# harskish/ganspace

Hardware: NVIDIA H100
Metric: latent samples/sec into PCA (StyleGAN2-ffhq W, N=1e6) (higher is better)
Workload: dtype f32

## Files before the change

### ganspace_b200/_native.py

```python
from __future__ import annotations

import contextlib
import ctypes as C
import os
from pathlib import Path

import torch

_LIB_PATH = Path(__file__).resolve().parent / "libganspace_b200.so"
_lib = None

_P, _I, _L, _Z, _D, _F = C.c_void_p, C.c_int, C.c_int64, C.c_size_t, C.c_double, C.c_float
SIGNATURES = {
    "gsb_abi_version": (_I, []),
    "gsb_last_error": (C.c_char_p, []),
    "gsb_legacy_normal_f32": (_I, [_P, _I, _L, _P, _L, _P]),
    "gsb_legacy_truncnorm_f32": (_I, [_P, _I, _L, _D, _D, _F, _P, _L, _P]),
    "gsb_mt19937_raw_u32": (_I, [_P, _I, _L, _P, _L, _P]),
    "gsb_mt19937_jump_polys": (_I, [_L, _I, _P]),
    "gsb_mt19937_jump_state_host": (_I, [C.c_uint32, _P, _P]),
    "gsb_legacy_normal_split_step_words": (_L, [_L, _I]),
    "gsb_legacy_normal_split_workspace_bytes": (_Z, [_I, _L, _I]),
    "gsb_legacy_normal_f32_split": (_I, [_P, _I, _L, _P, _L, _I, _P, _P, _Z, _P]),
    "gsb_legacy_normal_split_status": (_I, [_P, _I, _L, _I, _P, _P]),
    "gsb_mapping_packed_bytes": (_Z, [_I, _I]),
    "gsb_mapping_pack": (_I, [_P, _P, _I, _I, _F, _P, _P]),
    "gsb_mapping_workspace_bytes": (_Z, [_L, _I]),
    "gsb_mapping_forward": (_I, [_P, _I, _I, _P, _P, _L, _I, _P, _Z, _P]),
    "gsb_mapping_status": (_I, [_P, _I, _I, _P]),
    "gsb_linear_forward": (_I, [_P, _P, _P, _P, _L, _I, _I, _I, _P, _Z, _P]),
    "gsb_linear_workspace_bytes": (_Z, [_L, _I, _I, _I]),
    "gsb_batch_stats_workspace_bytes": (_Z, [_L, _I]),
    "gsb_batch_stats": (_I, [_P, _L, _I, _L, _P, _P, _P, _Z, _P]),
    "gsb_batch_stats_multi_workspace_bytes": (_Z, [_I, _L, _I]),
    "gsb_batch_stats_multi": (_I, [_P, _I, _L, _I, _L, _P, _P, _P, _Z, _P]),
    "gsb_ipca_state_bytes": (_Z, [_I, _I]),
    "gsb_ipca_workspace_bytes": (_Z, [_I, _I]),
    "gsb_ipca_reset": (_I, [_P, _I, _I, _P]),
    "gsb_ipca_chain_step": (_I, [_P, _I, _I, _L, _L, _P, _P, _P, _Z, _P]),
    "gsb_ipca_export": (_I, [_P, _I, _I, _L, _P, _P, _P, _P, _P, _P, _P]),
    "gsb_sym_eig_top": (_I, [_P, _I, _I, _P, _P, _P, _Z, _P]),
    "gsb_eig_status": (_I, [_P, _P]),
    "gsb_project_std_workspace_bytes": (_Z, [_I]),
    "gsb_project_std": (_I, [_P, _L, _I, _L, _P, _I, _P, _P, _P, _Z, _P]),
    "gsb_linreg_state_bytes": (_Z, [_I, _I]),
    "gsb_linreg_reset": (_I, [_P, _I, _I, _P]),
    "gsb_linreg_workspace_bytes": (_Z, [_L, _I]),
    "gsb_linreg_accumulate": (_I, [_P, _I, _I, _P, _L, _I, _P, _P, _P, _P, _P, _Z, _P]),
    "gsb_linreg_solve": (_I, [_P, _I, _I, _L, _P, _P, _P]),
    "gsb_linreg_solve_status": (_I, [_P, _I, _I, _P, _P]),
    "gsb_linreg_normal_matrix": (_P, [_P, _I, _I]),
    "gsb_linreg_solve_pinv": (_I, [_P, _I, _I, _P, _P, _D, _P, _P]),
    "gsb_ipca_set_chain_mode": (_I, [_I]),
    "gsb_synthesis_packed_bytes": (_Z, [_P, _I, _I]),
    "gsb_synthesis_pack": (_I, [_P, _I, _I, _P, _P, _Z, _P]),
    "gsb_synthesis_workspace_bytes": (_Z, [_P, _I, _L]),
    "gsb_synthesis_forward": (_I, [_P, _P, _I, _I, _I, _P, _L, _P, _L, _P, _Z, _P]),
    "gsb_synthesis_status": (_I, [_P, _P, _I, _I, _P]),
    "gsb_synthesis_render_workspace_bytes": (_Z, [_P, _I, _L, _I]),
    "gsb_synthesis_render": (_I, [_P, _P, _I, _I, _I, _P, _I, _P, _I, _L, _P, _L, _P, _P, _Z, _P]),
    "gsb_bigd_rows": (_I, [_I, _I]),
    "gsb_bigd_state_bytes": (_Z, [_L, _I]),
# ... 359 lines not shown
    return mean_out, gram_out


def batch_stats_multi(x: torch.Tensor, n_groups: int, rows_per_group: int, mean_out: torch.Tensor = None,
                      gram_out: torch.Tensor = None):
    lib = load()
    assert x.is_cuda and x.dtype == torch.float32 and x.dim() == 2 and x.stride(1) == 1
    assert x.shape[0] >= n_groups * rows_per_group
    d, ld = x.shape[1], x.stride(0)
    mean = mean_out if mean_out is not None else torch.empty((n_groups, d), dtype=torch.float64, device=x.device)
    gram = gram_out if gram_out is not None else torch.empty((n_groups, d, d), dtype=torch.float64, device=x.device)
    assert mean.shape == (n_groups, d) and gram.shape == (n_groups, d, d) and mean.dtype == gram.dtype == torch.float64
    ws_bytes = lib.gsb_batch_stats_multi_workspace_bytes(n_groups, rows_per_group, d)
    ws = scratch.get("stats", ws_bytes, x.device)
    with torch.cuda.device(x.device), instrument.section("stats"):
        _check(lib.gsb_batch_stats_multi(C.c_void_p(x.data_ptr()), n_groups, rows_per_group, d, ld, _ptr(mean), _ptr(gram),
                                         _ptr(ws), ws.numel(), _stream()), "gsb_batch_stats_multi")
    instrument.count(4 if (d % 128 == 0 and d <= 1024) else 3 * n_groups)
    return mean, gram


class IPCAChain:

    def __init__(self, d: int, c: int, device, side_stream: bool = True):
        lib = load()
        self.dev = require_cuda(device)
        self.d, self.c = int(d), int(c)
        self.state = torch.empty(lib.gsb_ipca_state_bytes(self.d, self.c), dtype=torch.uint8, device=self.dev)
        self.ws = torch.empty(lib.gsb_ipca_workspace_bytes(self.d, self.c), dtype=torch.uint8, device=self.dev)
        self.n_seen = 0
        self.stream = None
        if side_stream and os.environ.get("GANSPACE_B200_CHAIN_STREAM", "1") != "0":
            with torch.cuda.device(self.dev):
                self.stream = torch.cuda.Stream(device=self.dev, priority=-1)
        with torch.cuda.device(self.dev):
            _check(lib.gsb_ipca_reset(_ptr(self.state), self.d, self.c, _stream()), "gsb_ipca_reset")
            if self.stream is not None:
                self.stream.wait_stream(torch.cuda.current_stream())

    def step(self, n_batch: int, mean_b: torch.Tensor, gram_b: torch.Tensor):
        lib = load()
        assert mean_b.dtype == torch.float64 and gram_b.dtype == torch.float64
        with torch.cuda.device(self.dev):
            if self.stream is not None:
                self.stream.wait_stream(torch.cuda.current_stream())
                mean_b.record_stream(self.stream)
                gram_b.record_stream(self.stream)
                ctx = torch.cuda.stream(self.stream)
            else:
                ctx = contextlib.nullcontext()
            with ctx, instrument.section("chain"):
                _check(lib.gsb_ipca_chain_step(_ptr(self.state), self.d, self.c, self.n_seen, int(n_batch),
                                               _ptr(mean_b), _ptr(gram_b), _ptr(self.ws), self.ws.numel(), _stream()),
                       "gsb_ipca_chain_step")
        subspace = (self.d % 128 == 0 and 128 <= self.d <= 512 and self.c % 8 == 0 and 8 <= self.c <= 128
                    and os.environ.get("GANSPACE_B200_CHAIN", "") != "direct" and not _chain_forced_direct)
        instrument.count((1 if self.n_seen > 0 else 9) if subspace else 8)
        self.n_seen += int(n_batch)

    def join(self):
        if self.stream is not None:
            with torch.cuda.device(self.dev):
                torch.cuda.current_stream().wait_stream(self.stream)

    def export(self):
        lib = load()
        self.join()
        f64 = dict(dtype=torch.float64, device=self.dev)
        out = {
            "components": torch.empty((self.c, self.d), **f64), "singular_values": torch.empty(self.c, **f64),
            "mean": torch.empty(self.d, **f64), "var": torch.empty(self.d, **f64),
            "explained_variance": torch.empty(self.c, **f64),
            "explained_variance_ratio": torch.empty(self.c, **f64),
        }
        with torch.cuda.device(self.dev):
            _check(lib.gsb_ipca_export(_ptr(self.state), self.d, self.c, self.n_seen, _ptr(out["components"]),
                                       _ptr(out["singular_values"]), _ptr(out["mean"]), _ptr(out["var"]),
                                       _ptr(out["explained_variance"]), _ptr(out["explained_variance_ratio"]),
                                       _stream()), "gsb_ipca_export")
            check_eig_status("IPCAChain.export")
        instrument.count(1)
# ... 395 lines not shown
```

### ganspace_b200/csrc/ipca.cu

```cuda
#include "ipca_internal.cuh"
#include <math.h>

namespace gsb {

constexpr int ST_HDR = 24;

struct StateView {
    double *hdr, *mean, *unnorm, *S, *V;
    double *H, *Qbuf;
    void *eig_ws;
    size_t bytes;
};
static inline size_t export_eig_n(int c) { return (size_t)(c + 31) / 32 * 32; }
inline StateView state_view(void *p, int d, int c) {
    StateView s;
    s.hdr = reinterpret_cast<double *>(p);
    s.mean = s.hdr + ST_HDR;
    s.unnorm = s.mean + d;
    s.S = s.unnorm + d;
    s.V = s.S + c;
    size_t off = align_up((size_t)(ST_HDR + 2 * (size_t)d + c + (size_t)c * d) * sizeof(double), 256);
    s.H = s.Qbuf = nullptr; s.eig_ws = nullptr;
    if (subspace_applicable(d, c)) {
        char *b = reinterpret_cast<char *>(p);
// ... 129 lines not shown
extern "C" int gsb_ipca_chain_step(void *d_state, int d, int c, int64_t n_seen, int64_t n_batch,
                                   const double *d_mean_b, const double *d_gram_b, void *d_workspace,
                                   size_t workspace_bytes, gsb_stream_t stream) {
    GSB_CHECK_ARG(d_state && d_mean_b && d_gram_b && d_workspace, "ipca_chain_step: null pointer");
    if (int r = gsb::check_dims(d, c)) return r;
    GSB_CHECK_ARG(n_seen >= 0 && n_batch > 0, "ipca_chain_step: bad counts");
    GSB_CHECK_ARG(n_seen > 0 || c <= n_batch, "ipca_chain_step: n_components=%d > first batch size %lld", c,
                  (long long)n_batch);
    gsb::Workspace w = gsb::carve(d_workspace, d, c);
    if (workspace_bytes < w.bytes) {
        gsb::set_error("ipca_chain_step: workspace too small (%zu < %zu)", workspace_bytes, w.bytes);
        return GSB_ERR_WORKSPACE;
    }
    cudaStream_t st = (cudaStream_t)stream;
    gsb::StateView s = gsb::state_view(d_state, d, c);
    const bool subspace = gsb::subspace_applicable(d, c);
    if (subspace && n_seen > 0) {
        const size_t off = w.bytes;
        gsb::SubspaceWs sw = gsb::carve_subspace(reinterpret_cast<char *>(d_workspace) + off, d, c);
        if (workspace_bytes < off + sw.bytes) {
            gsb::set_error("ipca_chain_step: workspace too small (%zu < %zu)", workspace_bytes, off + sw.bytes);
            return GSB_ERR_WORKSPACE;
        }
        return gsb::subspace_step(s.hdr, s.mean, s.unnorm, s.H, s.Qbuf, d_mean_b, d_gram_b, sw, d, c, (double)n_seen,
                                  (double)n_batch, st);
    }
    dim3 grid((d + 31) / 32, (d + 31) / 32), block(32, 8);
    gsb::build_g_kernel<<<grid, block, 0, st>>>(d_gram_b, d_mean_b, s.mean, s.S, s.V, d, c, (double)n_seen,
                                                (double)n_batch, w.A);
    GSB_CHECK_LAUNCH();
    if (int r = gsb::eig_top(w, d, c, w.lam, w.evecs, st)) return r;
    size_t tot = (size_t)c * d;
    gsb::finalize_kernel<<<(unsigned)((tot + 255) / 256), 256, 0, st>>>(
        s.hdr, s.mean, s.unnorm, s.S, s.V, d_mean_b, d_gram_b, w.lam, w.evecs, d, c, (double)n_seen,
        (double)n_batch);
    GSB_CHECK_LAUNCH();
    if (subspace) return gsb::to_subspace_form(s.hdr, s.S, s.V, s.H, s.Qbuf, d, c, st);
    return GSB_OK;
}

extern "C" int gsb_ipca_set_chain_mode(int mode) {
    GSB_CHECK_ARG(mode == 0 || mode == 1, "ipca_set_chain_mode: mode must be 0 or 1");
    gsb::g_chain_force_direct = mode;
    return GSB_OK;
}

extern "C" int gsb_ipca_export(const void *d_state, int d, int c, int64_t n_seen, double *d_components,
                               double *d_singular_values, double *d_mean, double *d_var,
                               double *d_explained_variance, double *d_explained_variance_ratio,
                               gsb_stream_t stream) {
    GSB_CHECK_ARG(d_state, "ipca_export: null state");
    if (int r = gsb::check_dims(d, c)) return r;
    GSB_CHECK_ARG(n_seen > 1, "ipca_export: nothing fitted yet");
    gsb::StateView s = gsb::state_view(const_cast<void *>(d_state), d, c);
    if (gsb::subspace_applicable(d, c)) {
        if (int r = gsb::materialise_components(s.hdr, s.S, s.V, s.H, s.Qbuf, s.eig_ws, d, c, (cudaStream_t)stream)) return r;
    }
    gsb::export_kernel<<<1, 1024, 0, (cudaStream_t)stream>>>(s.hdr, s.mean, s.unnorm, s.S, s.V, d, c,
                                                            (double)n_seen, d_components, d_singular_values,
                                                            d_mean, d_var, d_explained_variance,
                                                            d_explained_variance_ratio);
    GSB_CHECK_LAUNCH();
    return GSB_OK;
// ... 13 lines not shown
```

### ganspace_b200/csrc/ipca_internal.cuh

```cuda
#pragma once
#include "eig.cuh"

namespace gsb {

int *eig_status_device_ptr();

struct SubspaceWs {
    double *Gt, *Part, *Red, *Slots;
    size_t bytes;
};
bool subspace_applicable(int d, int c);
bool chain_forced_direct();
size_t subspace_smem_bytes(int d, int c);
SubspaceWs carve_subspace(void *base, int d, int c);
int subspace_step(double *hdr, double *mean, double *unnorm, double *H, double *Qbuf, const double *mean_b, const double *gram_b,
                  const SubspaceWs &w, int d, int c, double n_seen, double n_b, cudaStream_t st);
int to_subspace_form(double *hdr, const double *S, const double *V, double *H, double *Qbuf, int d, int c, cudaStream_t st);
int materialise_components(double *hdr, double *S, double *V, const double *H, const double *Qbuf, void *eig_ws, int d, int c,
                           cudaStream_t st);

}
```

### ganspace_b200/csrc/subspace.cu

```cuda
#include "ipca_internal.cuh"
#include <math.h>
#include <stdlib.h>
#include <string.h>

namespace gsb {

constexpr int SC_CL = 16;
constexpr int SC_WARPS = 8;
constexpr int SC_THREADS = SC_WARPS * 32;
constexpr int SC_KT = 32;
constexpr int SC_LDA = SC_KT + 4;
constexpr int SC_STAGES = 3;
constexpr int SC_NB = 5;
constexpr int SC_MAXG = 2;

struct SubspaceParams {
    double *hdr, *mean, *unnorm, *H, *Qbuf;
    const double *mean_b, *gram_b;
    double *Gt, *Part, *Red, *Slots;
    double *Prof;
    int d, c;
    double n_seen, n_b, tol;
    double dbl;
    int maxit;
    int *status;
};

__device__ __forceinline__ void dmma884(double &c0, double &c1, double a, double b) {
    asm("mma.sync.aligned.m8n8k4.row.col.f64.f64.f64.f64 {%0,%1}, {%2}, {%3}, {%0,%1};" : "+d"(c0), "+d"(c1) : "d"(a), "d"(b));
}
__device__ __forceinline__ void sc_cluster_sync() {
    asm volatile("barrier.cluster.arrive.release.aligned;" ::: "memory");
    asm volatile("barrier.cluster.wait.acquire.aligned;" ::: "memory");
}
__device__ __forceinline__ void cp_async16(double *dst, const double *src) {
    const unsigned sa = (unsigned)__cvta_generic_to_shared(dst);
    asm volatile("cp.async.cg.shared.global [%0], [%1], 16;" ::"r"(sa), "l"(src) : "memory");
}
__device__ __forceinline__ void cta_copy_async(double *dst, const double *src, int ndoubles) {
    for (int ch = threadIdx.x; ch < ndoubles / 2; ch += SC_THREADS) cp_async16(dst + 2 * ch, src + 2 * ch);
}

template <bool AT, bool BT>
__device__ __forceinline__ void mma_group(const double *__restrict__ As, int lda, const double *__restrict__ Bs, int ldb,
                                          int ksteps, int m0, int n0, int nb, double (&acc)[SC_NB][2]) {
    const int lane = threadIdx.x & 31, g = lane >> 2, t = lane & 3;
    const double *ap = AT ? (As + (size_t)t * lda + m0 + g) : (As + (size_t)(m0 + g) * lda + t);
    const double *bp = BT ? (Bs + (size_t)(n0 + g) * ldb + t) : (Bs + (size_t)t * ldb + n0 + g);
// ... 142 lines not shown

template <int RA, int CB>
__global__ void __launch_bounds__(SC_THREADS, 1)
subspace_step_kernel(const SubspaceParams p) {
    extern __shared__ __align__(16) double sc_smem[];
    const int d = p.d, c = p.c, cp = c + 4, RPC = d / SC_CL, RT = RPC / 8, CT = c / 8, nkt = d / SC_KT;
    const int tid = threadIdx.x, lane = tid & 31, warp = tid >> 5, fg = lane >> 2, ft = lane & 3;
    uint32_t me_u;
    asm volatile("mov.u32 %0, %%cluster_ctarank;" : "=r"(me_u));
    const int me = (int)me_u;

    double *As = sc_smem;
    double *Bs = As + (size_t)SC_STAGES * RPC * SC_LDA;
    double *Ys = Bs + (size_t)SC_STAGES * SC_KT * cp;
    double *Qq = Ys + (size_t)RPC * cp;
    double *Ws = Qq + (size_t)RPC * cp;
    double *mv = Ws + (size_t)c * cp;
    double *red = mv + d;
    double *cholbuf = red + 64;
    long long tprev = clock64();
    double prof[10] = {0, 0, 0, 0, 0, 0, 0, 0, 0, 0};
#define PROF(k) do { const long long tn_ = clock64(); prof[k] += (double)(tn_ - tprev); tprev = tn_; } while (0)

    const double n_seen = p.n_seen, n_b = p.n_b, n_tot = n_seen + n_b;
    int cur = (int)__ldcg(p.hdr + 3);
    double *Qc = p.Qbuf + (size_t)cur * d * cp, *Qn = p.Qbuf + (size_t)(cur ^ 1) * d * cp;
    const size_t tileA = (size_t)RPC * SC_LDA, tileB = (size_t)SC_KT * cp;
    double *Gmine = p.Gt + (size_t)me * nkt * tileA;

    {
        const double f = sqrt((n_seen / n_tot) * n_b);
        for (int i = tid; i < d; i += SC_THREADS) mv[i] = f * (__ldcg(p.mean + i) - __ldcg(p.mean_b + i));
        const double *src = Qc + (size_t)me * RPC * cp;
        for (int i = tid; i < RPC * cp; i += SC_THREADS) Qq[i] = __ldcg(src + i);
        for (int i = tid; i < c * c; i += SC_THREADS) Ws[(i / c) * cp + i % c] = __ldcg(p.H + i);
    }
    __syncthreads();
    {
        const Grouping gr = make_grouping(RT, CT);
        for (int g = warp; g < gr.ngroups; g += SC_WARPS) {
            const int rt = g % gr.mt, ct0 = (g / gr.mt) * gr.nbsel;
            const int nb = (gr.nt - ct0 < gr.nbsel) ? gr.nt - ct0 : gr.nbsel;
            double acc[SC_NB][2];
            zero_acc(acc);
            mma_group<false, false>(Qq, cp, Ws, cp, c / 4, rt * 8, ct0 * 8, nb, acc);
#pragma unroll
            for (int b = 0; b < SC_NB; ++b)
                if (b < nb) {
                    double *o = Ys + (size_t)(rt * 8 + fg) * cp + (ct0 + b) * 8 + 2 * ft;
                    o[0] = acc[b][0]; o[1] = acc[b][1];
                }
        }
    }
    __syncthreads();
    PROF(0);
    {
        const Grouping gr = make_grouping(RT, SC_KT / 8);
        auto copy_c = [&](int stage, int kt_) {
            double *dstc = As + (size_t)stage * tileA;
            for (int ch = tid; ch < RPC * (SC_KT / 2); ch += SC_THREADS) {
                const int r = ch / (SC_KT / 2), o2 = ch % (SC_KT / 2);
                cp_async16(dstc + (size_t)r * SC_LDA + 2 * o2, p.gram_b + (size_t)(me * RPC + r) * d + kt_ * SC_KT + 2 * o2);
            }
        };
        for (int s = 0; s < SC_STAGES - 1; ++s) {
            if (s < nkt) { cta_copy_async(Bs + (size_t)s * tileB, Qc + (size_t)s * tileB, (int)tileB); copy_c(s, s); }
            asm volatile("cp.async.commit_group;" ::: "memory");
        }
        for (int kt = 0; kt < nkt; ++kt) {
            asm volatile("cp.async.wait_group %0;" ::"n"(SC_STAGES - 2) : "memory");
            __syncthreads();
            {
                const int nx = kt + SC_STAGES - 1;
                if (nx < nkt) {
                    cta_copy_async(Bs + (size_t)(nx % SC_STAGES) * tileB, Qc + (size_t)nx * tileB, (int)tileB);
                    copy_c(nx % SC_STAGES, nx);
                }
                asm volatile("cp.async.commit_group;" ::: "memory");
            }
            const double *Bt = Bs + (size_t)(kt % SC_STAGES) * tileB, *Cst = As + (size_t)(kt % SC_STAGES) * tileA;
            for (int g = warp; g < gr.ngroups; g += SC_WARPS) {
                const int rt = g % gr.mt, ct0 = (g / gr.mt) * gr.nbsel;
                const int nb = (gr.nt - ct0 < gr.nbsel) ? gr.nt - ct0 : gr.nbsel;
                double acc[SC_NB][2];
                zero_acc(acc);
// ... 171 lines not shown
            __syncthreads();
            partial_reduce();
            ++it;
            PROF(2);
        }
        for (int i = tid; i < c * c; i += SC_THREADS) Ws[(i / c) * cp + i % c] = __ldcg(p.Red + (size_t)c * c + i);
        __syncthreads();
        chol_solve_blocked<RA, CB>(Ws, Ys, c, cp, RPC, cholbuf);
        PROF(6);
        {
            double *dst = Qn + (size_t)me * RPC * cp;
            for (int i = tid; i < RPC * cp; i += SC_THREADS) {
                const double v = ((i % cp) < c) ? Ys[i] : 0.0;
                Qq[i] = v;
                dst[i] = v;
            }
        }
        __syncthreads();
        sc_cluster_sync();
        { double *t_ = Qc; Qc = Qn; Qn = t_; }
        cur ^= 1;
        PROF(7);
    }
    if (me == 0) {
        for (int i = tid; i < c * c; i += SC_THREADS) {
            const int a = i / c, b = i % c;
            p.H[i] = 0.5 * (Ws[(size_t)a * cp + b] + Ws[(size_t)b * cp + a]);
        }
    }
    for (int l = tid; l < RPC; l += SC_THREADS) {
        const int i = me * RPC + l;
        const double mb = __ldcg(p.mean_b + i), vb = __ldcg(p.gram_b + (size_t)i * d + i), mo = __ldcg(p.mean + i);
        const double r = n_seen / n_b;
        const double tq = (mo * n_seen) / r - mb * n_b;
        p.unnorm[i] = __ldcg(p.unnorm + i) + vb + r / n_tot * tq * tq;
        p.mean[i] = (mo * n_seen + mb * n_b) / n_tot;
    }
    __syncthreads();
    if (me == 0 && tid == 0) {
        p.hdr[0] = n_tot;
        p.hdr[1] += 1.0;
        p.hdr[2] = 1.0;
        p.hdr[3] = (double)cur;
        p.hdr[4] = (double)it;
        p.hdr[5] = rel;
        p.hdr[6] = fmax(p.hdr[6], rel);
        p.hdr[7] += (double)it;
        if (!conv) atomicOr(p.status, 2);
        PROF(8);
        for (int q = 0; q < 9; ++q) p.Prof[q] += prof[q];
        p.Prof[9] += (double)it;
        p.Prof[10] += 1.0;
    }
    __syncthreads();
    sc_cluster_sync();
}
#undef PROF

__global__ void to_subspace_kernel(double *hdr, const double *__restrict__ S, const double *__restrict__ V, double *__restrict__ H,
                                   double *__restrict__ Qbuf, int d, int c) {
    const int cp = c + 4;
    const size_t idx = blockIdx.x * (size_t)blockDim.x + threadIdx.x;
    if (idx < (size_t)d * cp) {
        const int i = (int)(idx / cp), t = (int)(idx % cp);
        Qbuf[idx] = (t < c) ? V[(size_t)t * d + i] : 0.0;
    }
    if (idx < (size_t)c * c) {
        const int a = (int)(idx / c), b = (int)(idx % c);
        H[idx] = (a == b) ? S[a] * S[a] : 0.0;
    }
    if (idx == 0) { hdr[2] = 1.0; hdr[3] = 0.0; hdr[4] = 0.0; hdr[5] = 0.0; hdr[6] = 0.0; hdr[7] = 0.0; }
}

__global__ void embed_h_kernel(const double *__restrict__ hdr, const double *__restrict__ H, int c, int n, double *__restrict__ A) {
    if (hdr[2] == 0.0) {
        for (int i = threadIdx.x; i < n * n; i += blockDim.x) A[i] = (i / n == i % n) ? -(double)(i / n + 1) : 0.0;
        return;
    }
// ... 69 lines not shown
    SubspaceWs w;
    char *p = reinterpret_cast<char *>(base);
    size_t off = 0;
    auto take = [&](size_t bytes) { char *q = p + off; off += align_up(bytes, 256); return q; };
    const int RPC = d / SC_CL, nkt = d / SC_KT;
    w.Gt = (double *)take((size_t)SC_CL * nkt * RPC * SC_LDA * 8);
    w.Part = (double *)take((size_t)SC_CL * 2 * c * c * 8);
    w.Red = (double *)take((size_t)2 * c * c * 8);
    w.Slots = (double *)take(SC_CL * 8);
    w.bytes = off;
    return w;
}

static double double_step_factor() {
    static double f = -1.0;
    if (f < 0.0) {
        const char *e = getenv("GANSPACE_B200_SUBSPACE_DBL");
        f = e ? atof(e) : 10.0;
        if (!(f > 0.0)) f = 1e300;
    }
    return f;
}

int subspace_step(double *hdr, double *mean, double *unnorm, double *H, double *Qbuf, const double *mean_b, const double *gram_b,
                  const SubspaceWs &w, int d, int c, double n_seen, double n_b, cudaStream_t st) {
    static double tol = -1.0;
    static int maxit = 0;
    if (tol < 0.0) {
        const char *e1 = getenv("GANSPACE_B200_SUBSPACE_TOL"), *e2 = getenv("GANSPACE_B200_SUBSPACE_MAXIT");
        tol = e1 ? atof(e1) : 1e-4;
        if (!(tol > 0.0)) tol = 1e-4;
        maxit = e2 ? atoi(e2) : 60;
        if (maxit < 1) maxit = 60;
    }
    const size_t smem = subspace_smem_bytes(d, c);
    const bool small = (c <= 80 && c + d / SC_CL <= 112);
    auto kern = small ? subspace_step_kernel<7, 5> : subspace_step_kernel<10, 8>;
    static bool cluster_set[2] = {false, false};
    if (!cluster_set[small]) {
        GSB_CHECK_CUDA(cudaFuncSetAttribute(kern, cudaFuncAttributeNonPortableClusterSizeAllowed, 1));
        cluster_set[small] = true;
    }
    if (int r = raise_dyn_smem(kern, smem)) return r;
    SubspaceParams p;
    p.hdr = hdr; p.mean = mean; p.unnorm = unnorm; p.H = H; p.Qbuf = Qbuf;
    p.mean_b = mean_b; p.gram_b = gram_b;
    p.Gt = w.Gt; p.Part = w.Part; p.Red = w.Red; p.Slots = w.Slots; p.Prof = hdr + 8;
    p.d = d; p.c = c; p.n_seen = n_seen; p.n_b = n_b; p.tol = tol; p.maxit = maxit; p.dbl = double_step_factor();
    p.status = eig_status_device_ptr();
    GSB_CHECK_ARG(p.status, "subspace_step: no device status word");
    cudaLaunchConfig_t cfg{};
    cfg.gridDim = dim3(SC_CL); cfg.blockDim = dim3(SC_THREADS); cfg.dynamicSmemBytes = smem; cfg.stream = st;
    cudaLaunchAttribute at[1];
    at[0].id = cudaLaunchAttributeClusterDimension;
    at[0].val.clusterDim.x = SC_CL; at[0].val.clusterDim.y = 1; at[0].val.clusterDim.z = 1;
    cfg.attrs = at; cfg.numAttrs = 1;
    GSB_CHECK_CUDA(cudaLaunchKernelEx(&cfg, kern, p));
    return GSB_OK;
}

int to_subspace_form(double *hdr, const double *S, const double *V, double *H, double *Qbuf, int d, int c, cudaStream_t st) {
    const size_t tot = (size_t)d * (c + 4);
    to_subspace_kernel<<<(unsigned)((tot + 255) / 256), 256, 0, st>>>(hdr, S, V, H, Qbuf, d, c);
    GSB_CHECK_LAUNCH();
    return GSB_OK;
}

int materialise_components(double *hdr, double *S, double *V, const double *H, const double *Qbuf, void *eig_ws, int d, int c,
                           cudaStream_t st) {
    const int n = (c + 31) / 32 * 32;
    Workspace w = carve(eig_ws, n, c);
    embed_h_kernel<<<1, 256, 0, st>>>(hdr, H, c, n, w.A);
    GSB_CHECK_LAUNCH();
    if (int r = eig_top(w, n, c, w.lam, w.evecs, st)) return r;
    GSB_CHECK_ARG(c <= 128, "materialise_components: c <= 128");
    rotate_kernel<<<dim3((unsigned)((d + 127) / 128), (unsigned)((c + ROT_T - 1) / ROT_T)), 128, 0, st>>>(hdr, w.evecs, n, w.lam, Qbuf, d,
                                                                                                    c, V, S);
    GSB_CHECK_LAUNCH();
    return sign_rows(V, c, d, st);
}
// ... 3 lines not shown
```

### ganspace_b200/decomposition.py

```python
from __future__ import annotations

import datetime
import inspect
import os
import sys
from pathlib import Path
from types import SimpleNamespace

import numpy as np
import torch

from . import _native
from . import plan as _plan
from .config import Config
from .estimators import get_estimator
from .models import get_instrumented_model
from .netdissect.nethook import InstrumentedModel

SEED_SAMPLING = 1
SEED_RANDOM_DIRS = 2
SEED_LINREG = 3
SEED_VISUALIZATION = 5

B = 20
# ... 35 lines not shown
    if dist.is_available() and dist.is_initialized() and dist.get_world_size() > 1:
        return dist.get_rank(), dist.get_world_size(), True
    return 0, 1, False


class _StatsExchange:

    def __init__(self, d, world):
        self.d, self.world = d, world

    def start(self, rnd, means, grams):
        import torch.distributed as dist
        g = means.shape[0]
        recv_m = torch.empty((self.world * g, self.d), dtype=torch.float64, device=means.device)
        recv_g = torch.empty((self.world * g, self.d, self.d), dtype=torch.float64, device=means.device)
        works = [dist.all_gather_into_tensor(recv_g, grams, async_op=True),
                 dist.all_gather_into_tensor(recv_m, means, async_op=True)]
        return rnd, g, recv_m, recv_g, works, (means, grams)

    def finish(self, pending, transformer, NB):
        rnd, g, recv_m, recv_g, works, _keep = pending
        for w in works:
            w.wait()
        for kk in rnd:
            slot = (kk % self.world) * g + (kk - rnd[0]) // self.world
            if not transformer.fit_partial_stats(NB, recv_m[slot], recv_g[slot]):
                return False
        return True


def _draw_seeds(count):
    hi = np.iinfo(np.int32).max
    return [int(np.random.randint(hi)) for _ in range(count)]


def _sample_batches(model, Bsz, seeds, out=None):
    if hasattr(model, "sample_latents_multi"):
        return model.sample_latents_multi(Bsz, seeds, out=out)
    return torch.cat([model.sample_latent(Bsz, seed=s) for s in seeds], dim=0)


def _sample_batches_lazy(model, Bsz, seeds):
    fn = getattr(model, "sample_latents_multi", None)
    if fn is not None and "lazy" in inspect.signature(fn).parameters:
        return fn(Bsz, seeds, lazy=True)
    return _sample_batches(model, Bsz, seeds), (lambda row_end: None)


def linreg_lstsq(comp_np, mean_np, stdev_np, inst, config, affine=None, native=False):
    print("Performing least squares regression", flush=True)
    torch.manual_seed(SEED_LINREG)
# ... 243 lines not shown
                    grams = torch.zeros((g_max, d, d), dtype=torch.float64, device=device) if (live and len(own) < g_max) \
                        else torch.empty((g_max, d, d), dtype=torch.float64, device=device)
                    if own:
                        k = own[0]
                        contiguous = all(where[own[i]] == where[own[0]] + i * NB for i in range(len(own)))
                        spans = [own] if contiguous else [[kk] for kk in own]
                        i0 = 0
                        for span in spans:
                            r0 = where[span[0]]
                            ensure_rows(r0 + len(span) * NB)
                            Xb = group_rows(lat[r0:r0 + len(span) * NB])
                            _native.batch_stats_multi(Xb, len(span), NB, mean_out=means[i0:i0 + len(span)],
                                                      gram_out=grams[i0:i0 + len(span)])
                            i0 += len(span)
                            if first is not None and span[0] * NB < first.shape[0]:
                                cnt = min(first.shape[0] - span[0] * NB, len(span) * NB)
                                first[span[0] * NB:span[0] * NB + cnt] = Xb[:cnt]
                        X = Xb[(len(span) - 1) * NB:]
                    if (K - 1) in rnd and _plan.owner(K - 1, world) != rank:
                        r0 = where[K - 1]
                        ensure_rows(r0 + NB)
                        X = group_rows(lat[r0:r0 + NB])
                    if exchange is None:
                        for i, kk in enumerate(own):
                            k = kk
                            if not transformer.fit_partial_stats(NB, means[i], grams[i]):
                                stop = True
                                break
                    else:
                        cur = exchange.start(rnd, means, grams)
                        if pending is not None and not exchange.finish(pending, transformer, NB):
                            stop = True
                        pending = cur
                        if rnd[0] < 2 * world * STATS_BLOCK and not stop:
                            if not exchange.finish(pending, transformer, NB):
                                stop = True
                            pending = None
                if pending is not None and not stop and not exchange.finish(pending, transformer, NB):
                    stop = True
            ensure_rows(lat.shape[0])
            del lat
    except KeyboardInterrupt:
        if live:
            raise
        if pooled:
            sys.exit(1)
        state["canceled_at"] = int(tr.n_samples_seen_)
    if pooled:
        if live:
            import torch.distributed as dist
            dist.all_reduce(first)
# ... 124 lines not shown
```

### ganspace_b200/estimators.py

```python
from __future__ import annotations

from types import SimpleNamespace

import numpy as np
import torch

from . import _native


class DeviceIncrementalPCA:

    def __init__(self, n_components, whiten=False, batch_size=None, device=None):
        if whiten:
            raise NotImplementedError("whiten=True is not used by GANSpace (estimators.py:58)")
        self.n_components = n_components
        self.whiten = whiten
        self.batch_size = batch_size
        self._device = device
        self._chain = None
        self._host = None
        self._dev = None
        self._shard = None
        self._stage = None
        self.n_samples_seen_ = np.int64(0)
# ... 48 lines not shown
        chain = self._chain
        if int(self.n_samples_seen_) == 0 and self.n_components > nb:
            raise ValueError(f"n_components={self.n_components} must be less or equal to the batch number of "
                             f"samples {nb} for the first partial_fit call.")
        if self._shard is not None:
            _native.exchange_rows(self._stage, chain.batch_rows(int(nb)), self._shard[1])
        chain.step(int(nb))
        self.n_samples_seen_ = np.int64(chain.n_seen)
        self._host = None
        return self

    def batch_stats(self, X):
        if isinstance(X, np.ndarray):
            dev = _native.require_cuda(self._device)
            X = torch.from_numpy(np.ascontiguousarray(X, dtype=np.float32)).to(dev)
        if X.dim() != 2:
            raise ValueError("Expected 2D array, got %dD" % X.dim())
        if X.dtype != torch.float32:
            X = X.float()
        mean, gram = _native.batch_stats(X)
        return int(X.shape[0]), mean, gram

    def merge(self, n_batch, mean_b, gram_b):
        chain = self._ensure(int(mean_b.shape[0]), mean_b.device)
        if int(self.n_samples_seen_) == 0 and self.n_components > n_batch:
            raise ValueError(f"n_components={self.n_components} must be less or equal to the batch number of "
                             f"samples {n_batch} for the first partial_fit call.")
        chain.step(n_batch, mean_b, gram_b)
        self.n_samples_seen_ = np.int64(chain.n_seen)
        self._host = None

    def partial_fit(self, X, y=None):
        d = int(X.shape[1]) if getattr(X, "ndim", 2) == 2 else 0
        if d > self.SMALL_D_MAX:
            if isinstance(X, np.ndarray):
                X = torch.from_numpy(np.ascontiguousarray(X, dtype=np.float32))
            dev = X.device if X.is_cuda else _native.require_cuda(self._device)
            self.batch_buffer(X.shape[0], d, dev).copy_(X)
            return self.partial_fit_inplace(X.shape[0])
        self.merge(*self.batch_stats(X))
        return self

    def last_batch_mean(self):
        return self._chain.gathered(self._chain.batch_mean.unsqueeze(0)).reshape(-1)

    def last_batch_rows(self, n):
        return self._chain.gathered(self._chain.batch_rows(self._chain.last_nb)[:n])

    def device_attributes(self):
        if self._chain is None:
            raise AttributeError("IncrementalPCA is not fitted yet")
        if self._host is None or self._dev is None:
            self._dev = self._chain.export()
# ... 183 lines not shown
```

### include/ganspace_b200.h

```cpp
#ifndef GANSPACE_B200_H
#define GANSPACE_B200_H

#include <stddef.h>
#include <stdint.h>

#ifdef __cplusplus
extern "C" {
#endif

#define GSB_ABI_VERSION 2

#define GSB_OK 0
#define GSB_ERR_ARG (-1)
#define GSB_ERR_CUDA (-2)
#define GSB_ERR_WORKSPACE (-3)

typedef void *gsb_stream_t;

int gsb_abi_version(void);
const char *gsb_last_error(void);

int gsb_legacy_normal_f32(const uint32_t *d_seeds, int n_streams, int64_t n_per_stream,
                          float *d_out, int64_t out_stride, gsb_stream_t stream);

// ... 21 lines not shown
int gsb_mapping_forward(const void *d_packed, int n_layers, int dim, const float *d_z, float *d_w,
                        int64_t n, int flags, void *d_workspace, size_t workspace_bytes,
                        gsb_stream_t stream);

size_t gsb_linear_workspace_bytes(int64_t n, int N, int K, int flags);
int gsb_linear_forward(const float *d_x, const float *d_w, const float *d_bias, float *d_y, int64_t n, int N,
                       int K, int flags, void *d_workspace, size_t workspace_bytes, gsb_stream_t stream);

int gsb_mapping_status(const void *d_packed, int n_layers, int dim, unsigned *h_flags);

size_t gsb_batch_stats_workspace_bytes(int64_t n, int d);
int gsb_batch_stats(const float *d_x, int64_t n, int d, int64_t ld, double *d_mean, double *d_gram,
                    void *d_workspace, size_t workspace_bytes, gsb_stream_t stream);
size_t gsb_batch_stats_multi_workspace_bytes(int n_groups, int64_t rows_per_group, int d);
int gsb_batch_stats_multi(const float *d_x, int n_groups, int64_t rows_per_group, int d, int64_t ld, double *d_mean,
                          double *d_gram, void *d_workspace, size_t workspace_bytes, gsb_stream_t stream);

size_t gsb_ipca_state_bytes(int d, int c);
size_t gsb_ipca_workspace_bytes(int d, int c);
int gsb_ipca_reset(void *d_state, int d, int c, gsb_stream_t stream);
int gsb_ipca_chain_step(void *d_state, int d, int c, int64_t n_seen, int64_t n_batch,
                        const double *d_mean_b, const double *d_gram_b,
                        void *d_workspace, size_t workspace_bytes, gsb_stream_t stream);
int gsb_ipca_export(const void *d_state, int d, int c, int64_t n_seen,
                    double *d_components, double *d_singular_values, double *d_mean, double *d_var,
                    double *d_explained_variance, double *d_explained_variance_ratio,
                    gsb_stream_t stream);

int gsb_sym_eig_top(double *d_a, int d, int c, double *d_evals, double *d_evecs,
                    void *d_workspace, size_t workspace_bytes, gsb_stream_t stream);

int gsb_eig_status(unsigned *h_flags, gsb_stream_t stream);

int gsb_ipca_set_chain_mode(int mode);

size_t gsb_project_std_workspace_bytes(int c);
int gsb_project_std(const float *d_x, int64_t n, int d, int64_t ld, const float *d_dirs, int c,
                    const double *d_sub, float *d_out_std, void *d_workspace, size_t workspace_bytes,
                    gsb_stream_t stream);

size_t gsb_linreg_state_bytes(int c, int latent_dim);
int gsb_linreg_reset(void *d_state, int c, int latent_dim, gsb_stream_t stream);
int gsb_linreg_accumulate(void *d_state, int c, int latent_dim, const float *d_act, int64_t n, int d,
                          const float *d_comp, const float *d_mean, const float *d_stdev,
                          const float *d_z, void *d_workspace, size_t workspace_bytes,
                          gsb_stream_t stream);
// ... 75 lines not shown
```

Before: 18.95 million.

## Batch multiple IPCA subspace chain steps into one persistent cluster kernel launch

Adds a multi-step chain entry point so that a round of per-batch mean/gram merges is deferred and then run as a single cluster kernel launch that loops over up to 64 steps. Between steps the Q and H state stay in shared memory instead of being reloaded from global memory, and H is written back only after the last step. This is meant to cut per-step launch overhead, Python call overhead and state reload traffic in the sequential IPCA chain. In exchange it adds round bookkeeping that identifies slots by pointer arithmetic, which is fragile, and each launch becomes longer and fully serial.

Result: faster. 19.47 million (median of 6 runs) (+2.8%).

```diff
diff --git a/ganspace_b200/_native.py b/ganspace_b200/_native.py
--- a/ganspace_b200/_native.py
+++ b/ganspace_b200/_native.py
@@ -38,6 +38,7 @@
     "gsb_ipca_workspace_bytes": (_Z, [_I, _I]),
     "gsb_ipca_reset": (_I, [_P, _I, _I, _P]),
     "gsb_ipca_chain_step": (_I, [_P, _I, _I, _L, _L, _P, _P, _P, _Z, _P]),
+    "gsb_ipca_chain_steps": (_I, [_P, _I, _I, _L, _L, _I, _P, _P, _P, _P, _Z, _P]),
     "gsb_ipca_export": (_I, [_P, _I, _I, _L, _P, _P, _P, _P, _P, _P, _P]),
     "gsb_sym_eig_top": (_I, [_P, _I, _I, _P, _P, _P, _Z, _P]),
     "gsb_eig_status": (_I, [_P, _P]),
@@ -443,6 +444,8 @@
 
 class IPCAChain:
 
+    ROUND_MAX = 64
+
     def __init__(self, d: int, c: int, device, side_stream: bool = True):
         lib = load()
         self.dev = require_cuda(device)
@@ -459,25 +462,48 @@
             if self.stream is not None:
                 self.stream.wait_stream(torch.cuda.current_stream())
 
-    def step(self, n_batch: int, mean_b: torch.Tensor, gram_b: torch.Tensor):
-        lib = load()
-        assert mean_b.dtype == torch.float64 and gram_b.dtype == torch.float64
+    def _enqueue(self, call, *tensors):
         with torch.cuda.device(self.dev):
             if self.stream is not None:
                 self.stream.wait_stream(torch.cuda.current_stream())
-                mean_b.record_stream(self.stream)
-                gram_b.record_stream(self.stream)
+                for t in tensors:
+                    t.record_stream(self.stream)
                 ctx = torch.cuda.stream(self.stream)
             else:
                 ctx = contextlib.nullcontext()
             with ctx, instrument.section("chain"):
-                _check(lib.gsb_ipca_chain_step(_ptr(self.state), self.d, self.c, self.n_seen, int(n_batch),
-                                               _ptr(mean_b), _ptr(gram_b), _ptr(self.ws), self.ws.numel(), _stream()),
-                       "gsb_ipca_chain_step")
-        subspace = (self.d % 128 == 0 and 128 <= self.d <= 512 and self.c % 8 == 0 and 8 <= self.c <= 128
-                    and os.environ.get("GANSPACE_B200_CHAIN", "") != "direct" and not _chain_forced_direct)
-        instrument.count((1 if self.n_seen > 0 else 9) if subspace else 8)
+                call()
+
+    def _subspace(self):
+        return (self.d % 128 == 0 and 128 <= self.d <= 512 and self.c % 8 == 0 and 8 <= self.c <= 128
+                and os.environ.get("GANSPACE_B200_CHAIN", "") != "direct" and not _chain_forced_direct)
+
+    def step(self, n_batch: int, mean_b: torch.Tensor, gram_b: torch.Tensor):
+        lib = load()
+        assert mean_b.dtype == torch.float64 and gram_b.dtype == torch.float64
+        self._enqueue(lambda: _check(lib.gsb_ipca_chain_step(_ptr(self.state), self.d, self.c, self.n_seen, int(n_batch),
+                                                             _ptr(mean_b), _ptr(gram_b), _ptr(self.ws), self.ws.numel(),
+                                                             _stream()), "gsb_ipca_chain_step"), mean_b, gram_b)
+        instrument.count((1 if self.n_seen > 0 else 9) if self._subspace() else 8)
         self.n_seen += int(n_batch)
+
+    def steps(self, n_batch: int, means: torch.Tensor, grams: torch.Tensor, slots):
+        lib = load()
+        d, g = self.d, len(slots)
+        assert g >= 1 and means.dtype == grams.dtype == torch.float64 and means.is_contiguous() and grams.is_contiguous()
+        assert means.dim() == 2 and means.shape[1] == d and grams.dim() == 3 and tuple(grams.shape[1:]) == (d, d)
+        assert all(0 <= s < means.shape[0] and s < grams.shape[0] for s in slots)
+        slot_arr = (C.c_int * g)(*[int(s) for s in slots])
+        self._enqueue(lambda: _check(lib.gsb_ipca_chain_steps(_ptr(self.state), d, self.c, self.n_seen, int(n_batch), g,
+                                                              _ptr(means), _ptr(grams), slot_arr, _ptr(self.ws),
+                                                              self.ws.numel(), _stream()), "gsb_ipca_chain_steps"),
+                      means, grams)
+        if self._subspace():
+            first = 1 if self.n_seen == 0 else 0
+            instrument.count(9 * first + -(-(g - first) // self.ROUND_MAX))
+        else:
+            instrument.count(8 * g)
+        self.n_seen += g * int(n_batch)
 
     def join(self):
         if self.stream is not None:
diff --git a/ganspace_b200/csrc/ipca.cu b/ganspace_b200/csrc/ipca.cu
--- a/ganspace_b200/csrc/ipca.cu
+++ b/ganspace_b200/csrc/ipca.cu
@@ -175,8 +175,9 @@
             gsb::set_error("ipca_chain_step: workspace too small (%zu < %zu)", workspace_bytes, off + sw.bytes);
             return GSB_ERR_WORKSPACE;
         }
-        return gsb::subspace_step(s.hdr, s.mean, s.unnorm, s.H, s.Qbuf, d_mean_b, d_gram_b, sw, d, c, (double)n_seen,
-                                  (double)n_batch, st);
+        const int slot0 = 0;
+        return gsb::subspace_steps(s.hdr, s.mean, s.unnorm, s.H, s.Qbuf, d_mean_b, d_gram_b, &slot0, 1, sw, d, c, (double)n_seen,
+                                   (double)n_batch, st);
     }
     dim3 grid((d + 31) / 32, (d + 31) / 32), block(32, 8);
     gsb::build_g_kernel<<<grid, block, 0, st>>>(d_gram_b, d_mean_b, s.mean, s.S, s.V, d, c, (double)n_seen,
@@ -192,6 +193,32 @@
     return GSB_OK;
 }
 
+extern "C" int gsb_ipca_chain_steps(void *d_state, int d, int c, int64_t n_seen, int64_t n_batch, int g, const double *d_means,
+                                    const double *d_grams, const int *slots, void *d_workspace, size_t workspace_bytes,
+                                    gsb_stream_t stream) {
+    GSB_CHECK_ARG(d_state && d_means && d_grams && slots && d_workspace, "ipca_chain_steps: null pointer");
+    if (int r = gsb::check_dims(d, c)) return r;
+    GSB_CHECK_ARG(g >= 1 && n_seen >= 0 && n_batch > 0, "ipca_chain_steps: bad counts");
+    for (int i = 0; i < g; ++i) GSB_CHECK_ARG(slots[i] >= 0, "ipca_chain_steps: negative slot %d at step %d", slots[i], i);
+    const bool subspace = gsb::subspace_applicable(d, c);
+    int i = 0;
+    for (; i < g && (!subspace || n_seen + i * n_batch == 0); ++i) {
+        if (int r = gsb_ipca_chain_step(d_state, d, c, n_seen + i * n_batch, n_batch, d_means + (size_t)slots[i] * d,
+                                        d_grams + (size_t)slots[i] * d * d, d_workspace, workspace_bytes, stream))
+            return r;
+    }
+    if (i == g) return GSB_OK;
+    const size_t off = gsb::carve(d_workspace, d, c).bytes;
+    gsb::SubspaceWs sw = gsb::carve_subspace(reinterpret_cast<char *>(d_workspace) + off, d, c);
+    if (workspace_bytes < off + sw.bytes) {
+        gsb::set_error("ipca_chain_steps: workspace too small (%zu < %zu)", workspace_bytes, off + sw.bytes);
+        return GSB_ERR_WORKSPACE;
+    }
+    gsb::StateView s = gsb::state_view(d_state, d, c);
+    return gsb::subspace_steps(s.hdr, s.mean, s.unnorm, s.H, s.Qbuf, d_means, d_grams, slots + i, g - i, sw, d, c,
+                               (double)(n_seen + i * n_batch), (double)n_batch, (cudaStream_t)stream);
+}
+
 extern "C" int gsb_ipca_set_chain_mode(int mode) {
     GSB_CHECK_ARG(mode == 0 || mode == 1, "ipca_set_chain_mode: mode must be 0 or 1");
     gsb::g_chain_force_direct = mode;
diff --git a/ganspace_b200/csrc/ipca_internal.cuh b/ganspace_b200/csrc/ipca_internal.cuh
--- a/ganspace_b200/csrc/ipca_internal.cuh
+++ b/ganspace_b200/csrc/ipca_internal.cuh
@@ -10,11 +10,12 @@
     size_t bytes;
 };
 bool subspace_applicable(int d, int c);
+constexpr int SC_ROUND_MAX = 64;
 bool chain_forced_direct();
 size_t subspace_smem_bytes(int d, int c);
 SubspaceWs carve_subspace(void *base, int d, int c);
-int subspace_step(double *hdr, double *mean, double *unnorm, double *H, double *Qbuf, const double *mean_b, const double *gram_b,
-                  const SubspaceWs &w, int d, int c, double n_seen, double n_b, cudaStream_t st);
+int subspace_steps(double *hdr, double *mean, double *unnorm, double *H, double *Qbuf, const double *means, const double *grams,
+                   const int *slots, int g, const SubspaceWs &w, int d, int c, double n_seen, double n_b, cudaStream_t st);
 int to_subspace_form(double *hdr, const double *S, const double *V, double *H, double *Qbuf, int d, int c, cudaStream_t st);
 int materialise_components(double *hdr, double *S, double *V, const double *H, const double *Qbuf, void *eig_ws, int d, int c,
                            cudaStream_t st);
diff --git a/ganspace_b200/csrc/subspace.cu b/ganspace_b200/csrc/subspace.cu
--- a/ganspace_b200/csrc/subspace.cu
+++ b/ganspace_b200/csrc/subspace.cu
@@ -16,7 +16,7 @@
 
 struct SubspaceParams {
     double *hdr, *mean, *unnorm, *H, *Qbuf;
-    const double *mean_b, *gram_b;
+    const double *means, *grams;
     double *Gt, *Part, *Red, *Slots;
     double *Prof;
     int d, c;
@@ -24,6 +24,8 @@
     double dbl;
     int maxit;
     int *status;
+    int nsteps;
+    int slot[SC_ROUND_MAX];
 };
 
 __device__ __forceinline__ void dmma884(double &c0, double &c1, double a, double b) {
@@ -212,18 +214,22 @@
     double prof[10] = {0, 0, 0, 0, 0, 0, 0, 0, 0, 0};
 #define PROF(k) do { const long long tn_ = clock64(); prof[k] += (double)(tn_ - tprev); tprev = tn_; } while (0)
 
-    const double n_seen = p.n_seen, n_b = p.n_b, n_tot = n_seen + n_b;
     int cur = (int)__ldcg(p.hdr + 3);
     double *Qc = p.Qbuf + (size_t)cur * d * cp, *Qn = p.Qbuf + (size_t)(cur ^ 1) * d * cp;
     const size_t tileA = (size_t)RPC * SC_LDA, tileB = (size_t)SC_KT * cp;
     double *Gmine = p.Gt + (size_t)me * nkt * tileA;
 
+  for (int step = 0; step < p.nsteps; ++step) {
+    const double n_b = p.n_b, n_seen = p.n_seen + step * n_b, n_tot = n_seen + n_b;
+    const double *mean_b = p.means + (size_t)p.slot[step] * d, *gram_b = p.grams + (size_t)p.slot[step] * d * d;
     {
         const double f = sqrt((n_seen / n_tot) * n_b);
-        for (int i = tid; i < d; i += SC_THREADS) mv[i] = f * (__ldcg(p.mean + i) - __ldcg(p.mean_b + i));
-        const double *src = Qc + (size_t)me * RPC * cp;
-        for (int i = tid; i < RPC * cp; i += SC_THREADS) Qq[i] = __ldcg(src + i);
-        for (int i = tid; i < c * c; i += SC_THREADS) Ws[(i / c) * cp + i % c] = __ldcg(p.H + i);
+        for (int i = tid; i < d; i += SC_THREADS) mv[i] = f * (__ldcg(p.mean + i) - __ldcg(mean_b + i));
+        if (step == 0) {
+            const double *src = Qc + (size_t)me * RPC * cp;
+            for (int i = tid; i < RPC * cp; i += SC_THREADS) Qq[i] = __ldcg(src + i);
+            for (int i = tid; i < c * c; i += SC_THREADS) Ws[(i / c) * cp + i % c] = __ldcg(p.H + i);
+        }
     }
     __syncthreads();
     {
@@ -250,7 +256,7 @@
             double *dstc = As + (size_t)stage * tileA;
             for (int ch = tid; ch < RPC * (SC_KT / 2); ch += SC_THREADS) {
                 const int r = ch / (SC_KT / 2), o2 = ch % (SC_KT / 2);
-                cp_async16(dstc + (size_t)r * SC_LDA + 2 * o2, p.gram_b + (size_t)(me * RPC + r) * d + kt_ * SC_KT + 2 * o2);
+                cp_async16(dstc + (size_t)r * SC_LDA + 2 * o2, gram_b + (size_t)(me * RPC + r) * d + kt_ * SC_KT + 2 * o2);
             }
         };
         for (int s = 0; s < SC_STAGES - 1; ++s) {
@@ -468,15 +474,22 @@
         cur ^= 1;
         PROF(7);
     }
-    if (me == 0) {
-        for (int i = tid; i < c * c; i += SC_THREADS) {
-            const int a = i / c, b = i % c;
-            p.H[i] = 0.5 * (Ws[(size_t)a * cp + b] + Ws[(size_t)b * cp + a]);
-        }
+    __syncthreads();
+    for (int i = tid; i < c * c; i += SC_THREADS) {
+        const int a = i / c, b = i % c;
+        if (a <= b) {
+            const double h = 0.5 * (Ws[(size_t)a * cp + b] + Ws[(size_t)b * cp + a]);
+            Ws[(size_t)a * cp + b] = h;
+            Ws[(size_t)b * cp + a] = h;
+        }
+    }
+    __syncthreads();
+    if (me == 0 && step == p.nsteps - 1) {
+        for (int i = tid; i < c * c; i += SC_THREADS) p.H[i] = Ws[(size_t)(i / c) * cp + i % c];
     }
     for (int l = tid; l < RPC; l += SC_THREADS) {
         const int i = me * RPC + l;
-        const double mb = __ldcg(p.mean_b + i), vb = __ldcg(p.gram_b + (size_t)i * d + i), mo = __ldcg(p.mean + i);
+        const double mb = __ldcg(mean_b + i), vb = __ldcg(gram_b + (size_t)i * d + i), mo = __ldcg(p.mean + i);
         const double r = n_seen / n_b;
         const double tq = (mo * n_seen) / r - mb * n_b;
         p.unnorm[i] = __ldcg(p.unnorm + i) + vb + r / n_tot * tq * tq;
@@ -494,12 +507,13 @@
         p.hdr[7] += (double)it;
         if (!conv) atomicOr(p.status, 2);
         PROF(8);
-        for (int q = 0; q < 9; ++q) p.Prof[q] += prof[q];
+        for (int q = 0; q < 9; ++q) { p.Prof[q] += prof[q]; prof[q] = 0.0; }
         p.Prof[9] += (double)it;
         p.Prof[10] += 1.0;
     }
     __syncthreads();
     sc_cluster_sync();
+  }
 }
 #undef PROF
 
@@ -615,8 +629,8 @@
     return f;
 }
 
-int subspace_step(double *hdr, double *mean, double *unnorm, double *H, double *Qbuf, const double *mean_b, const double *gram_b,
-                  const SubspaceWs &w, int d, int c, double n_seen, double n_b, cudaStream_t st) {
+int subspace_steps(double *hdr, double *mean, double *unnorm, double *H, double *Qbuf, const double *means, const double *grams,
+                   const int *slots, int g, const SubspaceWs &w, int d, int c, double n_seen, double n_b, cudaStream_t st) {
     static double tol = -1.0;
     static int maxit = 0;
     if (tol < 0.0) {
@@ -637,9 +651,9 @@
     if (int r = raise_dyn_smem(kern, smem)) return r;
     SubspaceParams p;
     p.hdr = hdr; p.mean = mean; p.unnorm = unnorm; p.H = H; p.Qbuf = Qbuf;
-    p.mean_b = mean_b; p.gram_b = gram_b;
+    p.means = means; p.grams = grams;
     p.Gt = w.Gt; p.Part = w.Part; p.Red = w.Red; p.Slots = w.Slots; p.Prof = hdr + 8;
-    p.d = d; p.c = c; p.n_seen = n_seen; p.n_b = n_b; p.tol = tol; p.maxit = maxit; p.dbl = double_step_factor();
+    p.d = d; p.c = c; p.n_b = n_b; p.tol = tol; p.maxit = maxit; p.dbl = double_step_factor();
     p.status = eig_status_device_ptr();
     GSB_CHECK_ARG(p.status, "subspace_step: no device status word");
     cudaLaunchConfig_t cfg{};
@@ -648,7 +662,12 @@
     at[0].id = cudaLaunchAttributeClusterDimension;
     at[0].val.clusterDim.x = SC_CL; at[0].val.clusterDim.y = 1; at[0].val.clusterDim.z = 1;
     cfg.attrs = at; cfg.numAttrs = 1;
-    GSB_CHECK_CUDA(cudaLaunchKernelEx(&cfg, kern, p));
+    for (int s0 = 0; s0 < g; s0 += SC_ROUND_MAX) {
+        p.nsteps = (g - s0 < SC_ROUND_MAX) ? g - s0 : SC_ROUND_MAX;
+        for (int s = 0; s < p.nsteps; ++s) p.slot[s] = slots[s0 + s];
+        p.n_seen = n_seen + s0 * n_b;
+        GSB_CHECK_CUDA(cudaLaunchKernelEx(&cfg, kern, p));
+    }
     return GSB_OK;
 }
 
diff --git a/ganspace_b200/decomposition.py b/ganspace_b200/decomposition.py
--- a/ganspace_b200/decomposition.py
+++ b/ganspace_b200/decomposition.py
@@ -1,5 +1,6 @@
 from __future__ import annotations
 
+import contextlib
 import datetime
 import inspect
 import os
@@ -81,11 +82,17 @@
         rnd, g, recv_m, recv_g, works, _keep = pending
         for w in works:
             w.wait()
-        for kk in rnd:
-            slot = (kk % self.world) * g + (kk - rnd[0]) // self.world
-            if not transformer.fit_partial_stats(NB, recv_m[slot], recv_g[slot]):
-                return False
+        with _merge_round(transformer, recv_m, recv_g):
+            for kk in rnd:
+                slot = (kk % self.world) * g + (kk - rnd[0]) // self.world
+                if not transformer.fit_partial_stats(NB, recv_m[slot], recv_g[slot]):
+                    return False
         return True
+
+
+def _merge_round(transformer, means, grams):
+    tr = getattr(transformer, "transformer", None)
+    return tr.round(means, grams) if hasattr(tr, "round") else contextlib.nullcontext()
 
 
 def _draw_seeds(count):
@@ -375,11 +382,12 @@
                         ensure_rows(r0 + NB)
                         X = group_rows(lat[r0:r0 + NB])
                     if exchange is None:
-                        for i, kk in enumerate(own):
-                            k = kk
-                            if not transformer.fit_partial_stats(NB, means[i], grams[i]):
-                                stop = True
-                                break
+                        with _merge_round(transformer, means, grams):
+                            for i, kk in enumerate(own):
+                                k = kk
+                                if not transformer.fit_partial_stats(NB, means[i], grams[i]):
+                                    stop = True
+                                    break
                     else:
                         cur = exchange.start(rnd, means, grams)
                         if pending is not None and not exchange.finish(pending, transformer, NB):
diff --git a/ganspace_b200/estimators.py b/ganspace_b200/estimators.py
--- a/ganspace_b200/estimators.py
+++ b/ganspace_b200/estimators.py
@@ -1,5 +1,6 @@
 from __future__ import annotations
 
+import contextlib
 from types import SimpleNamespace
 
 import numpy as np
@@ -94,6 +95,19 @@
         return int(X.shape[0]), mean, gram
 
     def merge(self, n_batch, mean_b, gram_b):
+        rnd = self._round
+        if rnd is not None:
+            slot = rnd.slot_of(mean_b, gram_b)
+            if slot is not None and (not rnd.slots or rnd.n_batch == int(n_batch)):
+                if int(self.n_samples_seen_) == 0 and self.n_components > n_batch:
+                    raise ValueError(f"n_components={self.n_components} must be less or equal to the batch number of "
+                                     f"samples {n_batch} for the first partial_fit call.")
+                rnd.n_batch = int(n_batch)
+                rnd.slots.append(slot)
+                self.n_samples_seen_ = np.int64(int(self.n_samples_seen_) + int(n_batch))
+                self._host = None
+                return
+            self._flush_round()
         chain = self._ensure(int(mean_b.shape[0]), mean_b.device)
         if int(self.n_samples_seen_) == 0 and self.n_components > n_batch:
             raise ValueError(f"n_components={self.n_components} must be less or equal to the batch number of "
@@ -101,6 +115,61 @@
         chain.step(n_batch, mean_b, gram_b)
         self.n_samples_seen_ = np.int64(chain.n_seen)
         self._host = None
+
+    def merge_many(self, n_batch, means, grams, slots):
+        if not len(slots):
+            return
+        chain = self._ensure(int(means.shape[1]), means.device)
+        if chain.n_seen == 0 and self.n_components > n_batch:
+            raise ValueError(f"n_components={self.n_components} must be less or equal to the batch number of "
+                             f"samples {n_batch} for the first partial_fit call.")
+        if hasattr(chain, "steps"):
+            chain.steps(int(n_batch), means, grams, list(slots))
+        else:
+            for s in slots:
+                chain.step(int(n_batch), means[s], grams[s])
+        self.n_samples_seen_ = np.int64(chain.n_seen)
+        self._host = None
+
+    class _Round:
+        def __init__(self, means, grams):
+            self.means, self.grams, self.slots, self.n_batch = means, grams, [], 0
+
+        def slot_of(self, mean_b, gram_b):
+            m, g = self.means, self.grams
+            if mean_b.device != m.device or mean_b.dtype != m.dtype or gram_b.dtype != g.dtype:
+                return None
+            d = m.shape[1]
+            om, og = mean_b.data_ptr() - m.data_ptr(), gram_b.data_ptr() - g.data_ptr()
+            i = om // (8 * d)
+            if om < 0 or om % (8 * d) or og != i * 8 * d * d or i >= m.shape[0] or i >= g.shape[0]:
+                return None
+            if tuple(mean_b.shape) != (d,) or tuple(gram_b.shape) != (d, d) or not (mean_b.is_contiguous() and
+                                                                                      gram_b.is_contiguous()):
+                return None
+            return int(i)
+
+    _round = None
+
+    def _flush_round(self):
+        rnd = self._round
+        if rnd is not None and rnd.slots:
+            slots, rnd.slots = rnd.slots, []
+            self.merge_many(rnd.n_batch, rnd.means, rnd.grams, slots)
+
+    @contextlib.contextmanager
+    def round(self, means, grams):
+        if means.dim() != 2 or grams.dim() != 3 or not (means.is_contiguous() and grams.is_contiguous()):
+            yield
+            return
+        self._round = self._Round(means, grams)
+        try:
+            yield
+        finally:
+            try:
+                self._flush_round()
+            finally:
+                self._round = None
 
     def partial_fit(self, X, y=None):
         d = int(X.shape[1]) if getattr(X, "ndim", 2) == 2 else 0
diff --git a/include/ganspace_b200.h b/include/ganspace_b200.h
--- a/include/ganspace_b200.h
+++ b/include/ganspace_b200.h
@@ -67,6 +67,9 @@
 int gsb_ipca_chain_step(void *d_state, int d, int c, int64_t n_seen, int64_t n_batch,
                         const double *d_mean_b, const double *d_gram_b,
                         void *d_workspace, size_t workspace_bytes, gsb_stream_t stream);
+int gsb_ipca_chain_steps(void *d_state, int d, int c, int64_t n_seen, int64_t n_batch, int g, const double *d_means,
+                         const double *d_grams, const int *slots, void *d_workspace, size_t workspace_bytes,
+                         gsb_stream_t stream);
 int gsb_ipca_export(const void *d_state, int d, int c, int64_t n_seen,
                     double *d_components, double *d_singular_values, double *d_mean, double *d_var,
                     double *d_explained_variance, double *d_explained_variance_ratio,
```
